# mit-han-lab/distrifuser

Measured on NVIDIA H100. Metric: SDXL 50-step latency (ms/image), lower is better.
Workload: dtype f16

## Files before the change

distrifuser_b200/_lib.py:

```python
from __future__ import annotations

import ctypes as C
import os

HERE = os.path.dirname(os.path.abspath(__file__))
LIB_PATH = os.environ.get("DF_LIB_PATH") or os.path.join(HERE, "libdistrifuser_b200.so")

NBANKS = 3
MAX_WORLD = 8
IPC_HANDLE_BYTES = 64
TENSORMAP_BYTES = 128

EXPORTS = (
    "df_last_error", "df_version", "df_device_sm_count", "df_symm_alloc", "df_symm_open", "df_symm_close",
    "df_symm_free", "df_step_begin", "df_slot_publish", "df_slot_wait", "df_groupnorm_scratch_bytes",
    "df_groupnorm_fwd", "df_groupnorm_halo_fwd", "df_halo_push", "df_halo_assemble", "df_attn_make_kvmaps", "df_attn_workspace_bytes", "df_attn_fwd",
    "df_output_gather", "df_output_gather_2d", "df_geglu", "df_add_layernorm", "df_bias_residual_add", "df_linear_supported", "df_linear_geglu_block", "df_linear_fwd",
)


class DfComm(C.Structure):
    _fields_ = [("base", C.c_void_p * MAX_WORLD), ("flags", C.c_void_p * MAX_WORLD), ("clock", C.c_void_p),
                ("tickets", C.c_void_p), ("bank_stride", C.c_uint64), ("spin_timeout_ns", C.c_uint64), ("world", C.c_int32),
                ("rank", C.c_int32)]


_lib = None


def lib():
    global _lib
    if _lib is None:
# ... 21 lines not shown
                                            u64, u64, u32, vp, i32, u64, u64, i32, i32, i32, i32, vp]
        L.df_halo_push.argtypes = [DfComm, vp, i32, i32, i32, i32, i32, u64, u64, i32, i32, vp]
        L.df_halo_assemble.argtypes = [DfComm, vp, vp, i32, i32, i32, i32, i32, u64, u64, i32, i32, i32, vp]
        L.df_attn_make_kvmaps.argtypes = [DfComm, u64, u64, i32, i32, i32, i32, vp, vp]
        L.df_attn_workspace_bytes.argtypes = [i32, i32, i32, i32, i32, i32]
        L.df_attn_workspace_bytes.restype = C.c_size_t
        L.df_attn_fwd.argtypes = [DfComm, vp, vp, vp, vp, i32, i32, i32, i32, i32, i64, i64, i64, i32, i32,
                                  C.POINTER(C.c_int32), i32, i32, f32, vp, C.c_size_t, vp]
        L.df_geglu.argtypes = [vp, vp, i64, i32, i64, i64, vp]
        L.df_add_layernorm.argtypes = [vp, vp, vp, vp, vp, vp, i64, i32, f32, vp]
        L.df_bias_residual_add.argtypes = [vp, vp, vp, vp, i64, i32, vp]
        L.df_linear_supported.argtypes = [i64, i32, i32, i32]
        L.df_linear_geglu_block.argtypes = [i64, i32, i32]
        L.df_linear_fwd.argtypes = [DfComm, vp, vp, vp, vp, vp, i64, i32, i32, i64, i64, i64, i64, i32, i32, i32, i32, i32, u32, u64,
                                    u64, i32, vp]
        L.df_output_gather.argtypes = [DfComm, vp, vp, i32, i32, i32, i32, i32, i32, i32, i32, i32, u64, vp]
        L.df_output_gather_2d.argtypes = [DfComm, vp, vp, i32, i32, i32, i32, i32, i32, i32, i32, i32, i32, i32, u64, vp]
        for name in EXPORTS:
            getattr(L, name)
        _lib = L
    return _lib


KERNELS_PER_CALL = {"df_groupnorm_fwd": 1, "df_groupnorm_halo_fwd": 1, "df_attn_fwd": 1, "df_halo_push": 1, "df_halo_assemble": 1,
                    "df_slot_publish": 1, "df_slot_wait": 1, "df_step_begin": 1, "df_output_gather": 2, "df_output_gather_2d": 2, "df_geglu": 1, "df_add_layernorm": 1, "df_bias_residual_add": 1,
                    "df_linear_fwd": 1}
LAUNCHES = {"total": 0}
PROFILE = None


# ... 11 lines not shown
```

distrifuser_b200/compat/unet_2d_condition.py:

```python
from __future__ import annotations

import math
from types import SimpleNamespace

import torch
from torch import nn
from torch.nn import functional as F

SDXL = dict(
    in_channels=4, out_channels=4, block_out_channels=(320, 640, 1280), layers_per_block=2,
    down_block_types=("DownBlock2D", "CrossAttnDownBlock2D", "CrossAttnDownBlock2D"),
    up_block_types=("CrossAttnUpBlock2D", "CrossAttnUpBlock2D", "UpBlock2D"),
    transformer_layers_per_block=(1, 2, 10), attention_head_dim=(5, 10, 20), cross_attention_dim=2048,
    use_linear_projection=True, norm_num_groups=32, norm_eps=1e-5, addition_embed_type="text_time",
    addition_time_embed_dim=256, projection_class_embeddings_input_dim=2816, sample_size=128,
)
SD15 = dict(
    in_channels=4, out_channels=4, block_out_channels=(320, 640, 1280, 1280), layers_per_block=2,
    down_block_types=("CrossAttnDownBlock2D",) * 3 + ("DownBlock2D",),
    up_block_types=("UpBlock2D",) + ("CrossAttnUpBlock2D",) * 3,
    transformer_layers_per_block=(1, 1, 1, 1), attention_head_dim=(8, 8, 8, 8), cross_attention_dim=768,
    use_linear_projection=False, norm_num_groups=32, norm_eps=1e-5, addition_embed_type=None,
    addition_time_embed_dim=None, projection_class_embeddings_input_dim=None, sample_size=64,
)
# ... 52 lines not shown
            if block:
                wi, bi = self._fused_weights(block)
                return ops.linear_geglu(x, wi, bi, block)
            return ops.geglu(self.proj(x))
        y = self.proj(x)
        x, gate = y.chunk(2, dim=-1)
        return x * F.gelu(gate)


class FeedForward(nn.Module):
    def __init__(self, dim):
        super().__init__()
        self.net = nn.ModuleList([GEGLU(dim, 4 * dim), nn.Dropout(0.0), nn.Linear(4 * dim, dim)])

    def forward(self, x):
        return self.net[2](self.net[0](x))


class BasicTransformerBlock(nn.Module):
    def __init__(self, dim, heads, head_dim, cross_dim):
        super().__init__()
        self.norm1 = nn.LayerNorm(dim)
        self.attn1 = Attention(dim, None, heads, head_dim)
        self.norm2 = nn.LayerNorm(dim)
        self.attn2 = Attention(dim, cross_dim, heads, head_dim)
        self.norm3 = nn.LayerNorm(dim)
        self.ff = FeedForward(dim)

    def forward_chained(self, x, pending, encoder_hidden_states=None):
        from ..ops import add_layernorm
        x, h = add_layernorm(x, pending, self.norm1)
# ... 18 lines not shown
        self.norm = nn.GroupNorm(groups, channels, eps=1e-6)
        self.proj_in = nn.Linear(channels, inner) if linear_proj else nn.Conv2d(channels, inner, 1)
        self.transformer_blocks = nn.ModuleList([BasicTransformerBlock(inner, heads, head_dim, cross_dim) for _ in range(depth)])
        self.proj_out = nn.Linear(inner, channels) if linear_proj else nn.Conv2d(inner, channels, 1)

    @staticmethod
    def _tokens(x):
        b, c, h, w = x.shape
        return x.permute(0, 2, 3, 1).reshape(b, h * w, c)

    @staticmethod
    def _image(t, h, w):
        b, _, c = t.shape
        return t.reshape(b, h, w, c).permute(0, 3, 1, 2)

    def forward(self, x, encoder_hidden_states=None):
        _, _, h, w = x.shape
        res = x
        x = self.norm(x)
        if self.use_linear_projection:
            t = self.proj_in(self._tokens(x))
        else:
            t = self._tokens(self.proj_in(x))
        if t.is_cuda and t.dtype == torch.float16:
            pending = None
            for blk in self.transformer_blocks:
                t, pending = blk.forward_chained(t, pending, encoder_hidden_states)
            t = t + pending
        else:
            for blk in self.transformer_blocks:
                t = blk(t, encoder_hidden_states=encoder_hidden_states)
        if self.use_linear_projection:
            x = self._image(self.proj_out(t), h, w)
        else:
            x = self.proj_out(self._image(t, h, w))
        return x + res


class ResnetBlock2D(nn.Module):
    def __init__(self, cin, cout, temb, groups, eps):
        super().__init__()
        self.norm1 = nn.GroupNorm(groups, cin, eps=eps)
        self.conv1 = nn.Conv2d(cin, cout, 3, padding=1)
        self.time_emb_proj = nn.Linear(temb, cout)
        self.norm2 = nn.GroupNorm(groups, cout, eps=eps)
        self.dropout = nn.Dropout(0.0)
        self.conv2 = nn.Conv2d(cout, cout, 3, padding=1)
        self.nonlinearity = nn.SiLU()
# ... 261 lines not shown
```

distrifuser_b200/csrc/common.cuh:

```cuda
#pragma once
#include <cuda.h>
#include <cuda_fp16.h>
#include <cuda_runtime.h>
#include <stdint.h>
#include <stdio.h>

#include "../../include/distrifuser_b200.h"

namespace df {

constexpr int kSmCount = 132;
int sm_count();

typedef CUresult (*EncodeTiledFn)(CUtensorMap*, CUtensorMapDataType, cuuint32_t, void*, const cuuint64_t*, const cuuint64_t*,
                                  const cuuint32_t*, const cuuint32_t*, CUtensorMapInterleave, CUtensorMapSwizzle,
                                  CUtensorMapL2promotion, CUtensorMapFloatOOBfill);
EncodeTiledFn tensor_map_encoder();

void set_error(const char* fmt, ...);

#define DF_CHECK_CUDA(expr)                                                              \
  do {                                                                                   \
    cudaError_t _e = (expr);                                                             \
    if (_e != cudaSuccess) {                                                             \
// ... 61 lines not shown
__device__ __forceinline__ int4 ld_v4(const void* p) {
  int4 r;
  asm volatile("ld.global.v4.s32 {%0,%1,%2,%3}, [%4];" : "=r"(r.x), "=r"(r.y), "=r"(r.z), "=r"(r.w) : "l"(p));
  return r;
}
__device__ __forceinline__ void st_v4(void* p, const int4& v) {
  asm volatile("st.global.v4.s32 [%0], {%1,%2,%3,%4};" ::"l"(p), "r"(v.x), "r"(v.y), "r"(v.z), "r"(v.w) : "memory");
}

unsigned pdl_mask();
enum { PDL_ATTN = 1, PDL_ELEM = 2, PDL_GN = 4, PDL_GEMM = 8 };

__device__ __forceinline__ void pdl_wait() { asm volatile("griddepcontrol.wait;" ::: "memory"); }

template <typename... KArgs, typename... Args>
inline cudaError_t launch_pdl(unsigned family, void (*kernel)(KArgs...), dim3 grid, dim3 block, size_t smem, cudaStream_t st, Args... args) {
  cudaLaunchConfig_t cfg = {};
  cfg.gridDim = grid;
  cfg.blockDim = block;
  cfg.dynamicSmemBytes = smem;
  cfg.stream = st;
  cudaLaunchAttribute attr[1];
  attr[0].id = cudaLaunchAttributeProgrammaticStreamSerialization;
  attr[0].val.programmaticStreamSerializationAllowed = (pdl_mask() & family) ? 1 : 0;
  cfg.attrs = attr;
  cfg.numAttrs = 1;
  return cudaLaunchKernelEx(&cfg, kernel, static_cast<KArgs>(args)...);
}


__host__ __device__ __forceinline__ uint64_t slot_offset(const df_comm_t& c, uint32_t epoch, uint64_t tensor_off,
                                                         uint64_t slot_bytes, int src) {
  return (uint64_t)(epoch % DF_NBANKS) * c.bank_stride + tensor_off + (uint64_t)src * slot_bytes;
}
__host__ __device__ __forceinline__ char* slot_ptr(const df_comm_t& c, int rank, uint32_t epoch, uint64_t tensor_off,
                                                   uint64_t slot_bytes, int src) {
  return (char*)c.base[rank] + slot_offset(c, epoch, tensor_off, slot_bytes, src);
}

__device__ __forceinline__ uint32_t* flag_ptr(const df_comm_t& c, int member, int idx, int src) {
  return c.flags[member] + (size_t)idx * c.world + src;
}
// ... 31 lines not shown
```

distrifuser_b200/csrc/linear.cu:

```cuda
#include <math.h>
#include <string.h>

#include "tc_ptx.cuh"

using namespace df;
using namespace df::tc;

namespace {

constexpr int BM = 128;
constexpr int BK = 64;
constexpr int NTHREADS = 288;
constexpr int NCONSUMER_WARPS = 8;
constexpr uint32_t A_BYTES = BM * BK * 2;

template <int BN> struct Stages { static constexpr int value = BN == 256 ? 4 : 5; };

template <int BN>
struct __align__(1024) SmemT {
  __half a[Stages<BN>::value][BM * BK];
  __half b[Stages<BN>::value][BN * BK];
  uint64_t full[Stages<BN>::value], empty[Stages<BN>::value];
};

// ... 15 lines not shown
  df_comm_t comm;
};

__device__ __forceinline__ float gelu_erf(float x) {
  const float z = fabsf(x) * 0.70710678118654752f;
  const float t = __fdividef(1.f, fmaf(0.3275911f, z, 1.f));
  float p = fmaf(1.061405429f, t, -1.453152027f);
  p = fmaf(p, t, 1.421413741f);
  p = fmaf(p, t, -0.284496736f);
  p = fmaf(p, t, 0.254829592f);
  const float e = p * t * __expf(-z * z);
  const float phi = x >= 0.f ? 1.f - 0.5f * e : 0.5f * e;
  return x * phi;
}

__device__ __forceinline__ float2 ld_h2f(const __half* p) { return __half22float2(*reinterpret_cast<const __half2*>(p)); }

template <int BN>
__device__ __forceinline__ void wgmma_tile(float* acc, uint64_t a_desc, uint64_t b_desc, uint32_t accumulate) {
  if constexpr (BN == 256) wgmma_ss_n256(acc, a_desc, b_desc, accumulate);
  else wgmma_ss_n160(acc, a_desc, b_desc, accumulate);
}

template <int EPI, int BN>
__global__ void __launch_bounds__(NTHREADS, 1)
linear_kernel(const __grid_constant__ CUtensorMap tm_a, const __grid_constant__ CUtensorMap tm_w, LinearArgs p) {
  static_assert(BN % 32 == 0 && BN <= 256 && (BN * BK * 2) % 1024 == 0, "tile shape");
  constexpr int STAGES = Stages<BN>::value;
  constexpr uint32_t B_BYTES = BN * BK * 2;
  using Smem = SmemT<BN>;
  extern __shared__ __align__(1024) uint8_t smem_raw[];
  Smem& sm = *reinterpret_cast<Smem*>(smem_raw);
  if ((smem_u32(smem_raw) & 1023u) != 0) __trap();
  const int warp = threadIdx.x >> 5, lane = threadIdx.x & 31;
  const int ntiles = p.tiles_m * p.tiles_n;
  const int kblocks = p.K / BK;

  if (threadIdx.x == 0) {
    for (int s = 0; s < STAGES; ++s) { mbar_init(&sm.full[s], 1); mbar_init(&sm.empty[s], NCONSUMER_WARPS); }
    asm volatile("fence.mbarrier_init.release.cluster;" ::: "memory");
  }
  __syncthreads();
  pdl_wait();

  if (warp == NCONSUMER_WARPS) {
    if (lane == 0) {
      prefetch_tmap(&tm_a);
      prefetch_tmap(&tm_w);
      uint32_t stage = 0, phase = 0;
      for (int tile = blockIdx.x; tile < ntiles; tile += gridDim.x) {
        const int tm = tile % p.tiles_m, tn = tile / p.tiles_m;
        for (int kb = 0; kb < kblocks; ++kb) {
          mbar_wait(&sm.empty[stage], phase ^ 1u);
          mbar_expect_tx(&sm.full[stage], A_BYTES + B_BYTES);
          tma_load_2d(sm.a[stage], &tm_a, &sm.full[stage], kb * BK, tm * BM);
          tma_load_2d(sm.b[stage], &tm_w, &sm.full[stage], kb * BK, tn * BN);
          if (++stage == STAGES) { stage = 0; phase ^= 1u; }
        }
      }
    }
  } else {
    const int wg = warp >> 2;
    const int c4 = lane & 3;
    const int rloc = wg * 64 + (warp & 3) * 16 + (lane >> 2);
    uint32_t pub_epoch = 0;
    if (p.publish) pub_epoch = p.comm.clock[0];
    uint32_t stage = 0, phase = 0;
    float acc[BN / 2];
    for (int tile = blockIdx.x; tile < ntiles; tile += gridDim.x) {
      const int tm = tile % p.tiles_m, tn = tile / p.tiles_m;
      fence_regs<BN / 2>(acc);
      uint32_t prev = 0;
      for (int kb = 0; kb < kblocks; ++kb) {
        mbar_wait(&sm.full[stage], phase);
        const uint32_t a_addr = smem_u32(sm.a[stage]) + wg * 64 * 128, b_addr = smem_u32(sm.b[stage]);
        wgmma_fence();
#pragma unroll
        for (int kk = 0; kk < BK / 16; ++kk)
          wgmma_tile<BN>(acc, smem_desc(a_addr + kk * 32, 16, 1024), smem_desc(b_addr + kk * 32, 16, 1024), (kb | kk) > 0);
        wgmma_commit();
        wgmma_wait<1>();
        if (kb > 0 && lane == 0) mbar_arrive(&sm.empty[prev]);
        prev = stage;
        if (++stage == STAGES) { stage = 0; phase ^= 1u; }
      }
      wgmma_wait<0>();
      fence_regs<BN / 2>(acc);
      if (lane == 0) mbar_arrive(&sm.empty[prev]);
#pragma unroll
      for (int h = 0; h < 2; ++h) {
        const int64_t grow = (int64_t)tm * BM + rloc + 8 * h;
        if (grow >= p.M) continue;
        if (EPI == EPI_GEGLU) {
          __half* dst = p.out + grow * p.ldo + tn * (BN / 2);
#pragma unroll
          for (int i = 0; i < BN / 16; ++i) {
            const int c = 8 * i + 2 * c4;
            float2 bh = make_float2(0.f, 0.f), bg = make_float2(0.f, 0.f);
            if (p.bias) { bh = ld_h2f(p.bias + tn * BN + c); bg = ld_h2f(p.bias + tn * BN + BN / 2 + c); }
            const float* hv = acc + 4 * i + 2 * h;
            const float* gv = acc + 4 * (i + BN / 16) + 2 * h;
            const float2 hf = __half22float2(__floats2half2_rn(hv[0] + bh.x, hv[1] + bh.y));
            const float2 gf = __half22float2(__floats2half2_rn(gv[0] + bg.x, gv[1] + bg.y));
            *reinterpret_cast<__half2*>(dst + c) = __floats2half2_rn(hf.x * gelu_erf(gf.x), hf.y * gelu_erf(gf.y));
          }
        } else {
          const int col0 = tn * BN;
          __half* dst = p.out + grow * p.ldo + col0;
          const __half* res = p.residual ? p.residual + grow * p.ldr + col0 : nullptr;
#pragma unroll
          for (int i = 0; i < BN / 8; ++i) {
            const int c = 8 * i + 2 * c4;
            const int col = col0 + c;
            if (col >= p.N) continue;
            float2 f = make_float2(acc[4 * i + 2 * h], acc[4 * i + 2 * h + 1]);
            if (p.bias) { const float2 bb = ld_h2f(p.bias + col); f.x += bb.x; f.y += bb.y; }
            __half2 o = __floats2half2_rn(f.x, f.y);
            if (res) o = __hadd2(o, *reinterpret_cast<const __half2*>(res + c));
            *reinterpret_cast<__half2*>(dst + c) = o;
            if (p.publish && col >= p.pub_col0) {
              const uint64_t off = slot_offset(p.comm, pub_epoch, p.tensor_off, p.slot_bytes, p.comm.rank) +
                                   ((uint64_t)grow * p.pub_cols + (col - p.pub_col0)) * 2;
              for (int q = 0; q < p.comm.world; ++q)
                if (p.peer_mask >> q & 1) *reinterpret_cast<__half2*>((char*)p.comm.base[q] + off) = o;
            }
          }
        }
      }
    }
  }
  if (p.publish) signal_when_last(p.comm, &p.comm.tickets[p.idx], gridDim.x, p.idx, p.peer_mask, p.comm.clock[0]);
}

int make_map2d(CUtensorMap* m, const void* base, int64_t rows, int K, int64_t pitch, int box_rows) {
  EncodeTiledFn enc = tensor_map_encoder();
  DF_REQUIRE(enc != nullptr, "cuTensorMapEncodeTiled is not available from this driver");
  cuuint64_t dims[2] = {(cuuint64_t)K, (cuuint64_t)rows};
  cuuint64_t strides[1] = {(cuuint64_t)pitch * 2};
  cuuint32_t box[2] = {BK, (cuuint32_t)box_rows};
  cuuint32_t estr[2] = {1, 1};
  CUresult r = enc(m, CU_TENSOR_MAP_DATA_TYPE_FLOAT16, 2, const_cast<void*>(base), dims, strides, box, estr,
                   CU_TENSOR_MAP_INTERLEAVE_NONE, CU_TENSOR_MAP_SWIZZLE_128B, CU_TENSOR_MAP_L2_PROMOTION_L2_256B,
                   CU_TENSOR_MAP_FLOAT_OOB_FILL_NONE);
  DF_REQUIRE(r == CUDA_SUCCESS, "cuTensorMapEncodeTiled failed (%d): base=%p rows=%lld K=%d pitch=%lld", (int)r, base,
             (long long)rows, K, (long long)pitch);
  return 0;
}

template <int EPI, int BN>
int launch_linear(const CUtensorMap& ta, const CUtensorMap& tw, const LinearArgs& args, int ctas, cudaStream_t st) {
  static bool attr_set = false;
  if (!attr_set) {
    DF_CHECK_CUDA(cudaFuncSetAttribute(linear_kernel<EPI, BN>, cudaFuncAttributeMaxDynamicSharedMemorySize, (int)sizeof(SmemT<BN>)));
    attr_set = true;
  }
  DF_CHECK_CUDA(launch_pdl(PDL_GEMM, linear_kernel<EPI, BN>, dim3(ctas), dim3(NTHREADS), sizeof(SmemT<BN>), st, ta, tw, args));
  return 0;
}

double tile_cost(int64_t M, int N, int bn, int ctas_avail) {
  const long long tm = (M + BM - 1) / BM, tn = (N + bn - 1) / bn, tiles = tm * tn;
  const long long rounds = (tiles + ctas_avail - 1) / ctas_avail;
  return (double)rounds * (bn + 64);
}

}

namespace {
int pick_bn(int64_t M, int N, int epilogue, int cap) {
  const bool ok160 = epilogue == EPI_PLAIN || N % 160 == 0, ok256 = epilogue == EPI_PLAIN || N % 256 == 0;
  if (!ok256) return ok160 ? 160 : 0;
  if (ok160 && tile_cost(M, N, 160, cap) < 0.97 * tile_cost(M, N, 256, cap)) return 160;
  return 256;
}
}

extern "C" int df_linear_supported(int64_t M, int N, int K, int epilogue) {
  if (M < 1 || N < 8 || N % 8 != 0 || K < BK || K % BK != 0) return 0;
  if (epilogue == EPI_GEGLU && pick_bn(M, N, epilogue, sm_count()) == 0) return 0;
  return 1;
}

extern "C" int df_linear_geglu_block(int64_t M, int N, int K) {
  (void)K;
  const int bn = pick_bn(M, N, EPI_GEGLU, sm_count());
  return bn / 2;
}

extern "C" int df_linear_fwd(df_comm_t comm, const void* a, const void* w, const void* bias, const void* residual, void* out,
                             int64_t M, int N, int K, int64_t lda, int64_t ldw, int64_t ldr, int64_t ldo, int epilogue,
                             int geglu_block, int publish, int pub_col0, int idx, uint32_t peer_mask, uint64_t tensor_off,
                             uint64_t slot_bytes, int max_ctas, void* stream) {
  DF_REQUIRE(epilogue == EPI_PLAIN || epilogue == EPI_GEGLU, "df_linear_fwd: unknown epilogue %d", epilogue);
  DF_REQUIRE(df_linear_supported(M, N, K, epilogue), "df_linear_fwd: unsupported shape M=%lld N=%d K=%d (N %% 8, K %% 64%s)",
             (long long)M, N, K, epilogue == EPI_GEGLU ? ", GEGLU: N % 256" : "");
  DF_REQUIRE(((uintptr_t)a % 16) == 0 && ((uintptr_t)w % 16) == 0 && ((uintptr_t)out % 16) == 0 && ((uintptr_t)bias % 16) == 0 &&
                 ((uintptr_t)residual % 16) == 0 && lda % 8 == 0 && ldw % 8 == 0 && ldo % 8 == 0 && ldr % 8 == 0,
             "df_linear_fwd: operands must be 16-byte aligned with pitches multiple of 8");
  DF_REQUIRE(!(publish && epilogue != EPI_PLAIN), "df_linear_fwd: publication is a plain-epilogue feature");
  LinearArgs args;
  memset(&args, 0, sizeof(args));
  args.bias = (const __half*)bias; args.residual = (const __half*)residual; args.out = (__half*)out;
  args.M = M; args.N = N; args.K = K; args.ldr = ldr; args.ldo = ldo;
  const int sms = sm_count();
  const int cap = max_ctas > 0 ? max_ctas : sms;
  int bn = pick_bn(M, N, epilogue, epilogue == EPI_GEGLU ? sms : cap);
  if (epilogue == EPI_GEGLU && geglu_block > 0) {
    DF_REQUIRE(geglu_block == 80 || geglu_block == 128, "df_linear_fwd: geglu_block must be 80 or 128");
    bn = 2 * geglu_block;
    DF_REQUIRE(N % bn == 0, "df_linear_fwd: interleave block %d does not tile N=%d", geglu_block, N);
  }
  args.tiles_m = (int)((M + BM - 1) / BM);
  args.tiles_n = (N + bn - 1) / bn;
  args.publish = publish && peer_mask != 0;
  args.comm = comm;
  if (args.publish) {
    DF_REQUIRE(pub_col0 >= 0 && pub_col0 < N && pub_col0 % 8 == 0, "df_linear_fwd: bad pub_col0");
    args.pub_col0 = pub_col0; args.pub_cols = N - pub_col0; args.idx = idx; args.peer_mask = peer_mask;
    args.tensor_off = tensor_off; args.slot_bytes = slot_bytes;
    DF_REQUIRE((uint64_t)M * args.pub_cols * 2 <= slot_bytes, "df_linear_fwd: published columns larger than the slot");
  }
  int ctas = args.tiles_m * args.tiles_n;
  if (ctas > cap) ctas = cap;
  if (ctas < 1) ctas = 1;
  CUtensorMap ta, tw;
  if (int rc = make_map2d(&ta, a, M, K, lda, BM)) return rc;
  if (int rc = make_map2d(&tw, w, N, K, ldw, bn)) return rc;
  cudaStream_t st = (cudaStream_t)stream;
  if (epilogue == EPI_GEGLU) {
    if (bn == 160) return launch_linear<EPI_GEGLU, 160>(ta, tw, args, ctas, st);
    return launch_linear<EPI_GEGLU, 256>(ta, tw, args, ctas, st);
  }
  if (bn == 160) return launch_linear<EPI_PLAIN, 160>(ta, tw, args, ctas, st);
  return launch_linear<EPI_PLAIN, 256>(ta, tw, args, ctas, st);
}
```

distrifuser_b200/csrc/tc_ptx.cuh:

```cuda
#pragma once
#include <cuda.h>

#include "common.cuh"

namespace df {
namespace tc {

__device__ __forceinline__ uint32_t smem_u32(const void* p) { return (uint32_t)__cvta_generic_to_shared(p); }

__device__ __forceinline__ void mbar_init(uint64_t* bar, uint32_t count) {
  asm volatile("mbarrier.init.shared::cta.b64 [%0], %1;" ::"r"(smem_u32(bar)), "r"(count));
}
__device__ __forceinline__ void mbar_expect_tx(uint64_t* bar, uint32_t bytes) {
  asm volatile("mbarrier.arrive.expect_tx.shared::cta.b64 _, [%0], %1;" ::"r"(smem_u32(bar)), "r"(bytes) : "memory");
}
__device__ __forceinline__ void mbar_arrive(uint32_t bar_addr) {
  asm volatile("mbarrier.arrive.shared::cta.b64 _, [%0];" ::"r"(bar_addr) : "memory");
}
__device__ __forceinline__ void mbar_arrive(uint64_t* bar) { mbar_arrive(smem_u32(bar)); }
#ifndef DF_TRYWAIT_HINT_NS
#define DF_TRYWAIT_HINT_NS 200000u
#endif
__device__ __forceinline__ bool mbar_try(uint32_t bar_addr, uint32_t parity) {
  uint32_t ok;
  asm volatile(
      "{\n\t.reg .pred p;\n\t"
      "mbarrier.try_wait.parity.shared::cta.b64 p, [%1], %2, %3;\n\t"
      "selp.u32 %0, 1, 0, p;\n\t}"
      : "=r"(ok)
      : "r"(bar_addr), "r"(parity), "r"(DF_TRYWAIT_HINT_NS)
      : "memory");
  return ok != 0;
}
__device__ __forceinline__ bool mbar_try(uint64_t* bar, uint32_t parity) { return mbar_try(smem_u32(bar), parity); }
// ... 16 lines not shown
  }
}

__device__ __forceinline__ void mbar_wait(uint64_t* bar, uint32_t parity) { mbar_wait(smem_u32(bar), parity); }

__device__ __forceinline__ void tma_load_4d(void* dst, const void* tmap, uint64_t* bar, int c0, int c1, int c2, int c3) {
  asm volatile(
      "cp.async.bulk.tensor.4d.shared::cluster.global.mbarrier::complete_tx::bytes [%0], [%1, {%3, %4, %5, %6}], [%2];"
      ::"r"(smem_u32(dst)), "l"((uint64_t)tmap), "r"(smem_u32(bar)), "r"(c0), "r"(c1), "r"(c2), "r"(c3)
      : "memory");
}
__device__ __forceinline__ void tma_load_2d(void* dst, const void* tmap, uint64_t* bar, int c0, int c1) {
  asm volatile(
      "cp.async.bulk.tensor.2d.shared::cluster.global.mbarrier::complete_tx::bytes [%0], [%1, {%3, %4}], [%2];"
      ::"r"(smem_u32(dst)), "l"((uint64_t)tmap), "r"(smem_u32(bar)), "r"(c0), "r"(c1)
      : "memory");
}
__device__ __forceinline__ void prefetch_tmap(const void* tmap) {
  asm volatile("prefetch.tensormap [%0];" ::"l"((uint64_t)tmap) : "memory");
}

__device__ __forceinline__ uint64_t smem_desc(uint32_t addr, uint32_t lbo_bytes, uint32_t sbo_bytes) {
  return (uint64_t)((addr & 0x3FFFFu) >> 4) | ((uint64_t)((lbo_bytes >> 4) & 0x3FFFu) << 16) |
         ((uint64_t)((sbo_bytes >> 4) & 0x3FFFu) << 32) | (1ull << 62);
}
__device__ __forceinline__ void wgmma_fence() { asm volatile("wgmma.fence.sync.aligned;" ::: "memory"); }
__device__ __forceinline__ void wgmma_commit() { asm volatile("wgmma.commit_group.sync.aligned;" ::: "memory"); }
template <int N>
__device__ __forceinline__ void wgmma_wait() { asm volatile("wgmma.wait_group.sync.aligned %0;" ::"n"(N) : "memory"); }
template <int N>
// ... 76 lines not shown
```

distrifuser_b200/modules/pp/attn.py:

```python
import ctypes as C
import os

import torch
from torch import nn
from torch.nn import functional as F

from ... import _lib
from ...utils import DistriConfig
from ..base_module import BaseModule, nvtx_range


_WORKSPACES: dict = {}


def _shared_workspace(device, nbytes: int) -> torch.Tensor:
    lst = _WORKSPACES.setdefault(device, [])
    if not lst or lst[-1].numel() < nbytes:
        if torch.cuda.is_current_stream_capturing():
            raise RuntimeError("attention workspace would grow during CUDA-graph capture; run one eager UNet call first")
        lst.append(torch.zeros(max(nbytes, 16 << 20), dtype=torch.uint8, device=device))
    return lst[-1]


class DistriAttentionPP(BaseModule):
# ... 35 lines not shown
            e0, e1 = torch.cuda.Event(enable_timing=True), torch.cuda.Event(enable_timing=True)
            e0.record()
        _lib.check(L.df_attn_fwd(comm, q.data_ptr(), kv_own.data_ptr(), out.data_ptr(), maps, b, lq, lseg,
                                 heads, d, q.stride(1), kv_own.stride(1), out.stride(1), nseg, own_seg,
                                 seg_rank, self.idx or 0, int(wait_flags), float(scale), ws, ws_bytes,
                                 torch.cuda.current_stream().cuda_stream), "df_attn_fwd")
        if prof is not None:
            e1.record()
            prof.append(dict(kernel="fmha_fwd_kernel", kind=kind,
                             flops=4.0 * b * lq * nseg * lseg * (real_width or Cq),
                             bytes=2.0 * (2 * b * lq * Cq + b * nseg * lseg * 2 * Cq),
                             shape=(b, lq, nseg * lseg, heads, d), start=e0, end=e1))
        return out

    def _project_out(self, hidden_states, residual, weight=None):
        attn = self.module
        if weight is not None:
            hidden_states = F.linear(hidden_states, weight, attn.to_out[0].bias)
        else:
            hidden_states = attn.to_out[0](hidden_states)
        hidden_states = attn.to_out[1](hidden_states)
        if attn.residual_connection:
            hidden_states = hidden_states + residual
        if attn.rescale_output_factor != 1.0:
            hidden_states = hidden_states / attn.rescale_output_factor
        return hidden_states


class DistriCrossAttentionPP(DistriAttentionPP):
    def __init__(self, module: nn.Module, distri_config: DistriConfig):
        super().__init__(module, distri_config)
        self.kv_cache = None

    @nvtx_range("DistriCrossAttentionPP")
    def forward(self, hidden_states, encoder_hidden_states=None, scale: float = 1.0, *args, **kwargs):
        assert encoder_hidden_states is not None
        self._require_cuda_half(hidden_states, "DistriCrossAttentionPP")
        attn = self.module
        q = attn.to_q(hidden_states)
        if self.counter == 0 or self.kv_cache is None:
            kv = self.to_kv(encoder_hidden_states)
            if self.kv_cache is not None and self.kv_cache.shape == kv.shape:
                self.kv_cache.copy_(kv)
            else:
                self.kv_cache = kv
        kv = self.kv_cache
        out = self._attend(q, kv, kv.shape[1], 1, 0, False, kind="cross")
        out = self._project_out(out, hidden_states)
        self.counter += 1
        return out


class DistriSelfAttentionPP(DistriAttentionPP):
    def __init__(self, module: nn.Module, distri_config: DistriConfig):
# ... 81 lines not shown
```

distrifuser_b200/ops.py:

```python
import os as _os

import torch

from . import _lib


def geglu(y: torch.Tensor) -> torch.Tensor:
    assert y.is_cuda and y.dtype == torch.float16 and y.stride(-1) == 1
    cols = y.shape[-1] // 2
    y2 = y.reshape(-1, 2 * cols)
    out = torch.empty((*y.shape[:-1], cols), dtype=y.dtype, device=y.device)
    _lib.check(_lib.lib().df_geglu(y2.data_ptr(), out.data_ptr(), y2.shape[0], cols, y2.stride(0), cols,
                                   torch.cuda.current_stream().cuda_stream), "df_geglu")
    return out


def add_layernorm(x: torch.Tensor, r: torch.Tensor | None, norm: torch.nn.LayerNorm):
    assert x.is_cuda and x.dtype == torch.float16
    C = x.shape[-1]
    x = x.contiguous()
    y = torch.empty_like(x)
    if r is not None:
        r = r.contiguous()
        s = torch.empty_like(x)
# ... 26 lines not shown
        out = out.contiguous(memory_format=torch.channels_last)
    if b is None or fold_bias:
        return residual + out
    if residual is not None:
        assert residual.shape == out.shape and residual.dtype == out.dtype
        if not residual.is_contiguous(memory_format=torch.channels_last):
            residual = residual.contiguous(memory_format=torch.channels_last)
    n, c, h, w = out.shape
    _lib.check(_lib.lib().df_bias_residual_add(out.data_ptr(), residual.data_ptr() if residual is not None else None,
                                               b.data_ptr(), out.data_ptr(), n * h * w, c,
                                               torch.cuda.current_stream().cuda_stream), "df_bias_residual_add")
    return out



_FUSED_LINEAR = set(_os.environ.get("DF_LINEAR", "geglu").replace("all", "geglu,qkv,out,ff2,proj").split(","))


def use_fused_linear(kind: str) -> bool:
    return kind in _FUSED_LINEAR


GEGLU_BLOCK = 128


def linear_supported(M: int, N: int, K: int, geglu: bool = False) -> bool:
    return bool(_lib.lib().df_linear_supported(M, N, K, 1 if geglu else 0))


def geglu_block(M: int, two_d: int, K: int) -> int:
    if not linear_supported(M, two_d, K, geglu=True):
        return 0
    return int(_lib.lib().df_linear_geglu_block(M, two_d, K))


# ... 47 lines not shown
```

include/distrifuser_b200.h:

```cpp
#ifndef DISTRIFUSER_B200_H
#define DISTRIFUSER_B200_H

#include <stddef.h>
#include <stdint.h>

#ifdef __cplusplus
extern "C" {
#endif

#define DF_NBANKS 3
#define DF_MAX_WORLD 8
#define DF_IPC_HANDLE_BYTES 64
#define DF_TENSORMAP_BYTES 128

const char* df_last_error(void);
int df_version(void);
int df_device_sm_count(int* out);

int df_symm_alloc(size_t bytes, void** dptr, void* ipc_handle_out_host );
int df_symm_open(const void* ipc_handle_host, void** peer_dptr);
int df_symm_close(void* peer_dptr);
int df_symm_free(void* dptr);

typedef struct {
// ... 49 lines not shown

int df_geglu(const void* in, void* out, int64_t rows, int cols, int64_t in_pitch, int64_t out_pitch, void* stream);

int df_bias_residual_add(const void* a, const void* residual , const void* bias, void* out, int64_t rows, int C,
                         void* stream);

int df_add_layernorm(const void* x, const void* r, void* s_out, void* y, const void* gamma, const void* beta,
                     int64_t rows, int C, float eps, void* stream);

int df_linear_supported(int64_t M, int N, int K, int epilogue);
int df_linear_geglu_block(int64_t M, int N, int K);
int df_linear_fwd(df_comm_t comm, const void* a, const void* w, const void* bias, const void* residual, void* out,
                  int64_t M, int N, int K, int64_t lda, int64_t ldw, int64_t ldr, int64_t ldo, int epilogue,
                  int geglu_block, int publish, int pub_col0, int idx, uint32_t peer_mask, uint64_t tensor_off,
                  uint64_t slot_bytes, int max_ctas, void* stream);

#ifdef __cplusplus
}
#endif
#endif
```

Before: 1561.

## Add 2-CTA cluster TMA multicast for GEMM weights and route more linears

Adds an optional 2-CTA cluster variant of the linear kernel where each CTA loads half of the weight tile and multicasts it to both CTAs, with cluster-wide empty-barrier release, to halve weight traffic from L2. It also adds a linear_layer helper that routes ff2, proj_in/proj_out (with fused residual), to_q and to_out through the custom kernel when their kinds are enabled. The cluster path is off unless DF_GEMM_CLUSTER=2, and DF_LINEAR still defaults to geglu only, so the new routing mostly falls back to torch by default. Bias loads switch to __ldg.

```diff
diff --git a/distrifuser_b200/_lib.py b/distrifuser_b200/_lib.py
--- a/distrifuser_b200/_lib.py
+++ b/distrifuser_b200/_lib.py
@@ -16,6 +16,7 @@
     "df_symm_free", "df_step_begin", "df_slot_publish", "df_slot_wait", "df_groupnorm_scratch_bytes",
     "df_groupnorm_fwd", "df_groupnorm_halo_fwd", "df_halo_push", "df_halo_assemble", "df_attn_make_kvmaps", "df_attn_workspace_bytes", "df_attn_fwd",
     "df_output_gather", "df_output_gather_2d", "df_geglu", "df_add_layernorm", "df_bias_residual_add", "df_linear_supported", "df_linear_geglu_block", "df_linear_fwd",
+    "df_linear_plan",
 )
 
 
@@ -67,6 +68,7 @@
         L.df_linear_geglu_block.argtypes = [i64, i32, i32]
         L.df_linear_fwd.argtypes = [DfComm, vp, vp, vp, vp, vp, i64, i32, i32, i64, i64, i64, i64, i32, i32, i32, i32, i32, u32, u64,
                                     u64, i32, vp]
+        L.df_linear_plan.argtypes = [i64, i32, i32, i32, i32, C.POINTER(i32), C.POINTER(i32), C.POINTER(i32)]
         L.df_output_gather.argtypes = [DfComm, vp, vp, i32, i32, i32, i32, i32, i32, i32, i32, i32, u64, vp]
         L.df_output_gather_2d.argtypes = [DfComm, vp, vp, i32, i32, i32, i32, i32, i32, i32, i32, i32, i32, i32, u64, vp]
         for name in EXPORTS:
diff --git a/distrifuser_b200/compat/unet_2d_condition.py b/distrifuser_b200/compat/unet_2d_condition.py
--- a/distrifuser_b200/compat/unet_2d_condition.py
+++ b/distrifuser_b200/compat/unet_2d_condition.py
@@ -90,7 +90,8 @@
         self.net = nn.ModuleList([GEGLU(dim, 4 * dim), nn.Dropout(0.0), nn.Linear(4 * dim, dim)])
 
     def forward(self, x):
-        return self.net[2](self.net[0](x))
+        from .. import ops
+        return ops.linear_layer(self.net[0](x), self.net[2], "ff2")
 
 
 class BasicTransformerBlock(nn.Module):
@@ -139,12 +140,19 @@
         b, _, c = t.shape
         return t.reshape(b, h, w, c).permute(0, 3, 1, 2)
 
+    def _project_out(self, t, res, h, w):
+        from .. import ops
+        if ops.use_fused_linear("proj") and res.is_cuda and res.is_contiguous(memory_format=torch.channels_last):
+            return self._image(ops.linear_layer(t, self.proj_out, "proj", residual=self._tokens(res)), h, w)
+        return self._image(self.proj_out(t), h, w) + res
+
     def forward(self, x, encoder_hidden_states=None):
         _, _, h, w = x.shape
         res = x
         x = self.norm(x)
         if self.use_linear_projection:
-            t = self.proj_in(self._tokens(x))
+            from .. import ops
+            t = ops.linear_layer(self._tokens(x), self.proj_in, "proj")
         else:
             t = self._tokens(self.proj_in(x))
         if t.is_cuda and t.dtype == torch.float16:
@@ -156,7 +164,7 @@
             for blk in self.transformer_blocks:
                 t = blk(t, encoder_hidden_states=encoder_hidden_states)
         if self.use_linear_projection:
-            x = self._image(self.proj_out(t), h, w)
+            return self._project_out(t, res, h, w)
         else:
             x = self.proj_out(self._image(t, h, w))
         return x + res
diff --git a/distrifuser_b200/csrc/common.cuh b/distrifuser_b200/csrc/common.cuh
--- a/distrifuser_b200/csrc/common.cuh
+++ b/distrifuser_b200/csrc/common.cuh
@@ -99,18 +99,31 @@
 __device__ __forceinline__ void pdl_wait() { asm volatile("griddepcontrol.wait;" ::: "memory"); }
 
 template <typename... KArgs, typename... Args>
-inline cudaError_t launch_pdl(unsigned family, void (*kernel)(KArgs...), dim3 grid, dim3 block, size_t smem, cudaStream_t st, Args... args) {
+inline cudaError_t launch_pdl_cluster(unsigned family, unsigned cluster, void (*kernel)(KArgs...), dim3 grid, dim3 block, size_t smem,
+                                      cudaStream_t st, Args... args) {
   cudaLaunchConfig_t cfg = {};
   cfg.gridDim = grid;
   cfg.blockDim = block;
   cfg.dynamicSmemBytes = smem;
   cfg.stream = st;
-  cudaLaunchAttribute attr[1];
+  cudaLaunchAttribute attr[2];
   attr[0].id = cudaLaunchAttributeProgrammaticStreamSerialization;
   attr[0].val.programmaticStreamSerializationAllowed = (pdl_mask() & family) ? 1 : 0;
   cfg.attrs = attr;
   cfg.numAttrs = 1;
+  if (cluster > 1) {
+    attr[1].id = cudaLaunchAttributeClusterDimension;
+    attr[1].val.clusterDim.x = cluster;
+    attr[1].val.clusterDim.y = 1;
+    attr[1].val.clusterDim.z = 1;
+    cfg.numAttrs = 2;
+  }
   return cudaLaunchKernelEx(&cfg, kernel, static_cast<KArgs>(args)...);
+}
+
+template <typename... KArgs, typename... Args>
+inline cudaError_t launch_pdl(unsigned family, void (*kernel)(KArgs...), dim3 grid, dim3 block, size_t smem, cudaStream_t st, Args... args) {
+  return launch_pdl_cluster(family, 1, kernel, grid, block, smem, st, args...);
 }
 
 
diff --git a/distrifuser_b200/csrc/linear.cu b/distrifuser_b200/csrc/linear.cu
--- a/distrifuser_b200/csrc/linear.cu
+++ b/distrifuser_b200/csrc/linear.cu
@@ -1,4 +1,5 @@
 #include <math.h>
+#include <stdlib.h>
 #include <string.h>
 
 #include "tc_ptx.cuh"
@@ -53,7 +54,7 @@
   return x * phi;
 }
 
-__device__ __forceinline__ float2 ld_h2f(const __half* p) { return __half22float2(*reinterpret_cast<const __half2*>(p)); }
+__device__ __forceinline__ float2 ld_bias(const __half* p) { return __half22float2(__ldg(reinterpret_cast<const __half2*>(p))); }
 
 template <int BN>
 __device__ __forceinline__ void wgmma_tile(float* acc, uint64_t a_desc, uint64_t b_desc, uint32_t accumulate) {
@@ -61,10 +62,22 @@
   else wgmma_ss_n160(acc, a_desc, b_desc, accumulate);
 }
 
-template <int EPI, int BN>
+template <int CLUSTER>
+__device__ __forceinline__ void release_stage(uint64_t* empty) {
+  if constexpr (CLUSTER == 1) {
+    mbar_arrive(empty);
+  } else {
+    const uint32_t addr = smem_u32(empty);
+#pragma unroll
+    for (uint32_t r = 0; r < CLUSTER; ++r) mbar_arrive_cluster(mapa_shared(addr, r));
+  }
+}
+
+template <int EPI, int BN, int CLUSTER>
 __global__ void __launch_bounds__(NTHREADS, 1)
 linear_kernel(const __grid_constant__ CUtensorMap tm_a, const __grid_constant__ CUtensorMap tm_w, LinearArgs p) {
   static_assert(BN % 32 == 0 && BN <= 256 && (BN * BK * 2) % 1024 == 0, "tile shape");
+  static_assert(CLUSTER == 1 || (CLUSTER == 2 && (BN / 2 * BK * 2) % 1024 == 0), "W half tile: whole 1 KiB swizzle atoms");
   constexpr int STAGES = Stages<BN>::value;
   constexpr uint32_t B_BYTES = BN * BK * 2;
   using Smem = SmemT<BN>;
@@ -72,14 +85,18 @@
   Smem& sm = *reinterpret_cast<Smem*>(smem_raw);
   if ((smem_u32(smem_raw) & 1023u) != 0) __trap();
   const int warp = threadIdx.x >> 5, lane = threadIdx.x & 31;
-  const int ntiles = p.tiles_m * p.tiles_n;
+  const uint32_t crank = CLUSTER == 1 ? 0u : cluster_ctarank();
+  const int tiles_mu = (p.tiles_m + CLUSTER - 1) / CLUSTER;
+  const int nunits = tiles_mu * p.tiles_n;
+  const int unit0 = blockIdx.x / CLUSTER, unit_step = gridDim.x / CLUSTER;
   const int kblocks = p.K / BK;
 
   if (threadIdx.x == 0) {
-    for (int s = 0; s < STAGES; ++s) { mbar_init(&sm.full[s], 1); mbar_init(&sm.empty[s], NCONSUMER_WARPS); }
+    for (int s = 0; s < STAGES; ++s) { mbar_init(&sm.full[s], 1); mbar_init(&sm.empty[s], NCONSUMER_WARPS * CLUSTER); }
     asm volatile("fence.mbarrier_init.release.cluster;" ::: "memory");
   }
-  __syncthreads();
+  if constexpr (CLUSTER == 1) __syncthreads();
+  else cluster_sync();
   pdl_wait();
 
   if (warp == NCONSUMER_WARPS) {
@@ -87,13 +104,17 @@
       prefetch_tmap(&tm_a);
       prefetch_tmap(&tm_w);
       uint32_t stage = 0, phase = 0;
-      for (int tile = blockIdx.x; tile < ntiles; tile += gridDim.x) {
-        const int tm = tile % p.tiles_m, tn = tile / p.tiles_m;
+      for (int u = unit0; u < nunits; u += unit_step) {
+        const int tm = (u % tiles_mu) * CLUSTER + (int)crank, tn = u / tiles_mu;
         for (int kb = 0; kb < kblocks; ++kb) {
           mbar_wait(&sm.empty[stage], phase ^ 1u);
           mbar_expect_tx(&sm.full[stage], A_BYTES + B_BYTES);
           tma_load_2d(sm.a[stage], &tm_a, &sm.full[stage], kb * BK, tm * BM);
-          tma_load_2d(sm.b[stage], &tm_w, &sm.full[stage], kb * BK, tn * BN);
+          if constexpr (CLUSTER == 1)
+            tma_load_2d(sm.b[stage], &tm_w, &sm.full[stage], kb * BK, tn * BN);
+          else
+            tma_load_2d_multicast(sm.b[stage] + crank * (BN / 2) * BK, &tm_w, &sm.full[stage], kb * BK,
+                                  tn * BN + (int)crank * (BN / 2), (uint16_t)((1u << CLUSTER) - 1));
           if (++stage == STAGES) { stage = 0; phase ^= 1u; }
         }
       }
@@ -106,8 +127,8 @@
     if (p.publish) pub_epoch = p.comm.clock[0];
     uint32_t stage = 0, phase = 0;
     float acc[BN / 2];
-    for (int tile = blockIdx.x; tile < ntiles; tile += gridDim.x) {
-      const int tm = tile % p.tiles_m, tn = tile / p.tiles_m;
+    for (int u = unit0; u < nunits; u += unit_step) {
+      const int tm = (u % tiles_mu) * CLUSTER + (int)crank, tn = u / tiles_mu;
       fence_regs<BN / 2>(acc);
       uint32_t prev = 0;
       for (int kb = 0; kb < kblocks; ++kb) {
@@ -119,13 +140,13 @@
           wgmma_tile<BN>(acc, smem_desc(a_addr + kk * 32, 16, 1024), smem_desc(b_addr + kk * 32, 16, 1024), (kb | kk) > 0);
         wgmma_commit();
         wgmma_wait<1>();
-        if (kb > 0 && lane == 0) mbar_arrive(&sm.empty[prev]);
+        if (kb > 0 && lane == 0) release_stage<CLUSTER>(&sm.empty[prev]);
         prev = stage;
         if (++stage == STAGES) { stage = 0; phase ^= 1u; }
       }
       wgmma_wait<0>();
       fence_regs<BN / 2>(acc);
-      if (lane == 0) mbar_arrive(&sm.empty[prev]);
+      if (lane == 0) release_stage<CLUSTER>(&sm.empty[prev]);
 #pragma unroll
       for (int h = 0; h < 2; ++h) {
         const int64_t grow = (int64_t)tm * BM + rloc + 8 * h;
@@ -136,7 +157,7 @@
           for (int i = 0; i < BN / 16; ++i) {
             const int c = 8 * i + 2 * c4;
             float2 bh = make_float2(0.f, 0.f), bg = make_float2(0.f, 0.f);
-            if (p.bias) { bh = ld_h2f(p.bias + tn * BN + c); bg = ld_h2f(p.bias + tn * BN + BN / 2 + c); }
+            if (p.bias) { bh = ld_bias(p.bias + tn * BN + c); bg = ld_bias(p.bias + tn * BN + BN / 2 + c); }
             const float* hv = acc + 4 * i + 2 * h;
             const float* gv = acc + 4 * (i + BN / 16) + 2 * h;
             const float2 hf = __half22float2(__floats2half2_rn(hv[0] + bh.x, hv[1] + bh.y));
@@ -153,7 +174,7 @@
             const int col = col0 + c;
             if (col >= p.N) continue;
             float2 f = make_float2(acc[4 * i + 2 * h], acc[4 * i + 2 * h + 1]);
-            if (p.bias) { const float2 bb = ld_h2f(p.bias + col); f.x += bb.x; f.y += bb.y; }
+            if (p.bias) { const float2 bb = ld_bias(p.bias + col); f.x += bb.x; f.y += bb.y; }
             __half2 o = __floats2half2_rn(f.x, f.y);
             if (res) o = __hadd2(o, *reinterpret_cast<const __half2*>(res + c));
             *reinterpret_cast<__half2*>(dst + c) = o;
@@ -169,6 +190,10 @@
     }
   }
   if (p.publish) signal_when_last(p.comm, &p.comm.tickets[p.idx], gridDim.x, p.idx, p.peer_mask, p.comm.clock[0]);
+  if constexpr (CLUSTER > 1) {
+    __syncwarp();
+    cluster_sync();
+  }
 }
 
 int make_map2d(CUtensorMap* m, const void* base, int64_t rows, int K, int64_t pitch, int box_rows) {
@@ -186,15 +211,52 @@
   return 0;
 }
 
+template <int EPI, int BN, int CLUSTER>
+int run_linear(const CUtensorMap* ta, const CUtensorMap* tw, const LinearArgs* args, int ctas, cudaStream_t st, int* max_clusters) {
+  static int clusters = 0;
+  if (clusters == 0) {
+    DF_CHECK_CUDA(cudaFuncSetAttribute(linear_kernel<EPI, BN, CLUSTER>, cudaFuncAttributeMaxDynamicSharedMemorySize,
+                                       (int)sizeof(SmemT<BN>)));
+    int n = 1;
+    if (CLUSTER > 1) {
+      cudaLaunchConfig_t cfg = {};
+      cfg.gridDim = dim3(CLUSTER * sm_count());
+      cfg.blockDim = dim3(NTHREADS);
+      cfg.dynamicSmemBytes = sizeof(SmemT<BN>);
+      cudaLaunchAttribute attr[1];
+      attr[0].id = cudaLaunchAttributeClusterDimension;
+      attr[0].val.clusterDim.x = CLUSTER;
+      attr[0].val.clusterDim.y = 1;
+      attr[0].val.clusterDim.z = 1;
+      cfg.attrs = attr;
+      cfg.numAttrs = 1;
+      DF_CHECK_CUDA(cudaOccupancyMaxActiveClusters(&n, linear_kernel<EPI, BN, CLUSTER>, &cfg));
+      DF_REQUIRE(n >= 1, "df_linear: no %d-CTA cluster of linear_kernel fits on the device", CLUSTER);
+    }
+    clusters = n;
+  }
+  if (max_clusters) *max_clusters = clusters;
+  if (ta == nullptr) return 0;
+  DF_CHECK_CUDA(launch_pdl_cluster(PDL_GEMM, CLUSTER, linear_kernel<EPI, BN, CLUSTER>, dim3(ctas), dim3(NTHREADS), sizeof(SmemT<BN>),
+                                   st, *ta, *tw, *args));
+  return 0;
+}
+
 template <int EPI, int BN>
-int launch_linear(const CUtensorMap& ta, const CUtensorMap& tw, const LinearArgs& args, int ctas, cudaStream_t st) {
-  static bool attr_set = false;
-  if (!attr_set) {
-    DF_CHECK_CUDA(cudaFuncSetAttribute(linear_kernel<EPI, BN>, cudaFuncAttributeMaxDynamicSharedMemorySize, (int)sizeof(SmemT<BN>)));
-    attr_set = true;
-  }
-  DF_CHECK_CUDA(launch_pdl(PDL_GEMM, linear_kernel<EPI, BN>, dim3(ctas), dim3(NTHREADS), sizeof(SmemT<BN>), st, ta, tw, args));
-  return 0;
+int run_linear(int cluster, const CUtensorMap* ta, const CUtensorMap* tw, const LinearArgs* args, int ctas, cudaStream_t st,
+               int* max_clusters) {
+  if (cluster == 2) return run_linear<EPI, BN, 2>(ta, tw, args, ctas, st, max_clusters);
+  return run_linear<EPI, BN, 1>(ta, tw, args, ctas, st, max_clusters);
+}
+
+int run_linear(int epilogue, int bn, int cluster, const CUtensorMap* ta, const CUtensorMap* tw, const LinearArgs* args, int ctas,
+               cudaStream_t st, int* max_clusters) {
+  if (epilogue == EPI_GEGLU) {
+    if (bn == 160) return run_linear<EPI_GEGLU, 160>(cluster, ta, tw, args, ctas, st, max_clusters);
+    return run_linear<EPI_GEGLU, 256>(cluster, ta, tw, args, ctas, st, max_clusters);
+  }
+  if (bn == 160) return run_linear<EPI_PLAIN, 160>(cluster, ta, tw, args, ctas, st, max_clusters);
+  return run_linear<EPI_PLAIN, 256>(cluster, ta, tw, args, ctas, st, max_clusters);
 }
 
 double tile_cost(int64_t M, int N, int bn, int ctas_avail) {
@@ -211,6 +273,43 @@
   if (!ok256) return ok160 ? 160 : 0;
   if (ok160 && tile_cost(M, N, 160, cap) < 0.97 * tile_cost(M, N, 256, cap)) return 160;
   return 256;
+}
+
+struct Plan {
+  int bn, cluster, ctas, tiles_m, tiles_n;
+};
+
+bool cluster_requested() {
+  const char* e = getenv("DF_GEMM_CLUSTER");
+  return e != nullptr && atoi(e) == 2;
+}
+
+int make_plan(int64_t M, int N, int epilogue, int geglu_block, int max_ctas, Plan* pl) {
+  const int sms = sm_count();
+  const int cap = max_ctas > 0 ? max_ctas : sms;
+  int bn = pick_bn(M, N, epilogue, epilogue == EPI_GEGLU ? sms : cap);
+  if (epilogue == EPI_GEGLU && geglu_block > 0) {
+    DF_REQUIRE(geglu_block == 80 || geglu_block == 128, "df_linear_fwd: geglu_block must be 80 or 128");
+    bn = 2 * geglu_block;
+    DF_REQUIRE(N % bn == 0, "df_linear_fwd: interleave block %d does not tile N=%d", geglu_block, N);
+  }
+  pl->bn = bn;
+  pl->tiles_m = (int)((M + BM - 1) / BM);
+  pl->tiles_n = (N + bn - 1) / bn;
+  pl->cluster = cluster_requested() && pl->tiles_m >= 2 && cap % 2 == 0 ? 2 : 1;
+  if (pl->cluster == 2) {
+    int max_clusters = 0;
+    if (int rc = run_linear(epilogue, bn, 2, nullptr, nullptr, nullptr, 0, nullptr, &max_clusters)) return rc;
+    long long clusters = (long long)((pl->tiles_m + 1) / 2) * pl->tiles_n;
+    if (clusters > max_clusters) clusters = max_clusters;
+    if (clusters > cap / 2) clusters = cap / 2;
+    pl->ctas = 2 * (int)clusters;
+  } else {
+    long long ctas = (long long)pl->tiles_m * pl->tiles_n;
+    if (ctas > cap) ctas = cap;
+    pl->ctas = ctas < 1 ? 1 : (int)ctas;
+  }
+  return 0;
 }
 }
 
@@ -241,16 +340,10 @@
   memset(&args, 0, sizeof(args));
   args.bias = (const __half*)bias; args.residual = (const __half*)residual; args.out = (__half*)out;
   args.M = M; args.N = N; args.K = K; args.ldr = ldr; args.ldo = ldo;
-  const int sms = sm_count();
-  const int cap = max_ctas > 0 ? max_ctas : sms;
-  int bn = pick_bn(M, N, epilogue, epilogue == EPI_GEGLU ? sms : cap);
-  if (epilogue == EPI_GEGLU && geglu_block > 0) {
-    DF_REQUIRE(geglu_block == 80 || geglu_block == 128, "df_linear_fwd: geglu_block must be 80 or 128");
-    bn = 2 * geglu_block;
-    DF_REQUIRE(N % bn == 0, "df_linear_fwd: interleave block %d does not tile N=%d", geglu_block, N);
-  }
-  args.tiles_m = (int)((M + BM - 1) / BM);
-  args.tiles_n = (N + bn - 1) / bn;
+  Plan pl;
+  if (int rc = make_plan(M, N, epilogue, geglu_block, max_ctas, &pl)) return rc;
+  args.tiles_m = pl.tiles_m;
+  args.tiles_n = pl.tiles_n;
   args.publish = publish && peer_mask != 0;
   args.comm = comm;
   if (args.publish) {
@@ -259,17 +352,19 @@
     args.tensor_off = tensor_off; args.slot_bytes = slot_bytes;
     DF_REQUIRE((uint64_t)M * args.pub_cols * 2 <= slot_bytes, "df_linear_fwd: published columns larger than the slot");
   }
-  int ctas = args.tiles_m * args.tiles_n;
-  if (ctas > cap) ctas = cap;
-  if (ctas < 1) ctas = 1;
   CUtensorMap ta, tw;
   if (int rc = make_map2d(&ta, a, M, K, lda, BM)) return rc;
-  if (int rc = make_map2d(&tw, w, N, K, ldw, bn)) return rc;
-  cudaStream_t st = (cudaStream_t)stream;
-  if (epilogue == EPI_GEGLU) {
-    if (bn == 160) return launch_linear<EPI_GEGLU, 160>(ta, tw, args, ctas, st);
-    return launch_linear<EPI_GEGLU, 256>(ta, tw, args, ctas, st);
-  }
-  if (bn == 160) return launch_linear<EPI_PLAIN, 160>(ta, tw, args, ctas, st);
-  return launch_linear<EPI_PLAIN, 256>(ta, tw, args, ctas, st);
-}
+  if (int rc = make_map2d(&tw, w, N, K, ldw, pl.bn / pl.cluster)) return rc;
+  return run_linear(epilogue, pl.bn, pl.cluster, &ta, &tw, &args, pl.ctas, (cudaStream_t)stream, nullptr);
+}
+
+extern "C" int df_linear_plan(int64_t M, int N, int K, int epilogue, int max_ctas, int* bn, int* cluster, int* ctas) {
+  DF_REQUIRE(epilogue == EPI_PLAIN || epilogue == EPI_GEGLU, "df_linear_plan: unknown epilogue %d", epilogue);
+  DF_REQUIRE(df_linear_supported(M, N, K, epilogue), "df_linear_plan: unsupported shape M=%lld N=%d K=%d", (long long)M, N, K);
+  Plan pl;
+  if (int rc = make_plan(M, N, epilogue, 0, max_ctas, &pl)) return rc;
+  *bn = pl.bn;
+  *cluster = pl.cluster;
+  *ctas = pl.ctas;
+  return 0;
+}
diff --git a/distrifuser_b200/csrc/tc_ptx.cuh b/distrifuser_b200/csrc/tc_ptx.cuh
--- a/distrifuser_b200/csrc/tc_ptx.cuh
+++ b/distrifuser_b200/csrc/tc_ptx.cuh
@@ -18,6 +18,23 @@
   asm volatile("mbarrier.arrive.shared::cta.b64 _, [%0];" ::"r"(bar_addr) : "memory");
 }
 __device__ __forceinline__ void mbar_arrive(uint64_t* bar) { mbar_arrive(smem_u32(bar)); }
+
+__device__ __forceinline__ uint32_t cluster_ctarank() {
+  uint32_t r;
+  asm volatile("mov.u32 %0, %%cluster_ctarank;" : "=r"(r));
+  return r;
+}
+__device__ __forceinline__ uint32_t mapa_shared(uint32_t addr, uint32_t rank) {
+  uint32_t r;
+  asm volatile("mapa.shared::cluster.u32 %0, %1, %2;" : "=r"(r) : "r"(addr), "r"(rank));
+  return r;
+}
+__device__ __forceinline__ void mbar_arrive_cluster(uint32_t cluster_addr) {
+  asm volatile("mbarrier.arrive.shared::cluster.b64 _, [%0];" ::"r"(cluster_addr) : "memory");
+}
+__device__ __forceinline__ void cluster_sync() {
+  asm volatile("barrier.cluster.arrive.release.aligned;\n\tbarrier.cluster.wait.acquire.aligned;" ::: "memory");
+}
 #ifndef DF_TRYWAIT_HINT_NS
 #define DF_TRYWAIT_HINT_NS 200000u
 #endif
@@ -64,6 +81,12 @@
   asm volatile(
       "cp.async.bulk.tensor.2d.shared::cluster.global.mbarrier::complete_tx::bytes [%0], [%1, {%3, %4}], [%2];"
       ::"r"(smem_u32(dst)), "l"((uint64_t)tmap), "r"(smem_u32(bar)), "r"(c0), "r"(c1)
+      : "memory");
+}
+__device__ __forceinline__ void tma_load_2d_multicast(void* dst, const void* tmap, uint64_t* bar, int c0, int c1, uint16_t cta_mask) {
+  asm volatile(
+      "cp.async.bulk.tensor.2d.shared::cluster.global.mbarrier::complete_tx::bytes.multicast::cluster [%0], [%1, {%3, %4}], [%2], %5;"
+      ::"r"(smem_u32(dst)), "l"((uint64_t)tmap), "r"(smem_u32(bar)), "r"(c0), "r"(c1), "h"(cta_mask)
       : "memory");
 }
 __device__ __forceinline__ void prefetch_tmap(const void* tmap) {
diff --git a/distrifuser_b200/modules/pp/attn.py b/distrifuser_b200/modules/pp/attn.py
--- a/distrifuser_b200/modules/pp/attn.py
+++ b/distrifuser_b200/modules/pp/attn.py
@@ -73,11 +73,9 @@
         return out
 
     def _project_out(self, hidden_states, residual, weight=None):
+        from ... import ops
         attn = self.module
-        if weight is not None:
-            hidden_states = F.linear(hidden_states, weight, attn.to_out[0].bias)
-        else:
-            hidden_states = attn.to_out[0](hidden_states)
+        hidden_states = ops.linear_layer(hidden_states, attn.to_out[0], "out", weight=weight)
         hidden_states = attn.to_out[1](hidden_states)
         if attn.residual_connection:
             hidden_states = hidden_states + residual
@@ -95,8 +93,9 @@
     def forward(self, hidden_states, encoder_hidden_states=None, scale: float = 1.0, *args, **kwargs):
         assert encoder_hidden_states is not None
         self._require_cuda_half(hidden_states, "DistriCrossAttentionPP")
+        from ... import ops
         attn = self.module
-        q = attn.to_q(hidden_states)
+        q = ops.linear_layer(hidden_states, attn.to_q, "q")
         if self.counter == 0 or self.kv_cache is None:
             kv = self.to_kv(encoder_hidden_states)
             if self.kv_cache is not None and self.kv_cache.shape == kv.shape:
diff --git a/distrifuser_b200/ops.py b/distrifuser_b200/ops.py
--- a/distrifuser_b200/ops.py
+++ b/distrifuser_b200/ops.py
@@ -64,11 +64,26 @@
 
 
 
-_FUSED_LINEAR = set(_os.environ.get("DF_LINEAR", "geglu").replace("all", "geglu,qkv,out,ff2,proj").split(","))
+_FUSED_LINEAR = set(_os.environ.get("DF_LINEAR", "geglu").replace("all", "geglu,qkv,out,q,ff2,proj").split(","))
 
 
 def use_fused_linear(kind: str) -> bool:
     return kind in _FUSED_LINEAR
+
+
+def linear_layer(x: torch.Tensor, layer: torch.nn.Linear, kind: str, weight: torch.Tensor | None = None,
+                 residual: torch.Tensor | None = None) -> torch.Tensor:
+    import torch.nn.functional as F
+    w = layer.weight if weight is None else weight
+    b = layer.bias
+    plain = type(layer).forward is torch.nn.Linear.forward
+    if (use_fused_linear(kind) and plain and x.is_cuda and x.dtype == torch.float16 and w.dtype == torch.float16 and
+            x.stride(-1) == 1 and w.is_contiguous() and (b is None or (b.dtype == torch.float16 and b.is_contiguous())) and
+            (residual is None or (residual.dtype == torch.float16 and residual.stride(-1) == 1)) and
+            linear_supported(x.numel() // x.shape[-1], w.shape[0], w.shape[1])):
+        return linear(x, w, b, residual)
+    y = layer(x) if weight is None else F.linear(x, w, b)
+    return y if residual is None else y + residual
 
 
 GEGLU_BLOCK = 128
diff --git a/include/distrifuser_b200.h b/include/distrifuser_b200.h
--- a/include/distrifuser_b200.h
+++ b/include/distrifuser_b200.h
@@ -87,6 +87,7 @@
                   int64_t M, int N, int K, int64_t lda, int64_t ldw, int64_t ldr, int64_t ldo, int epilogue,
                   int geglu_block, int publish, int pub_col0, int idx, uint32_t peer_mask, uint64_t tensor_off,
                   uint64_t slot_bytes, int max_ctas, void* stream);
+int df_linear_plan(int64_t M, int N, int K, int epilogue, int max_ctas, int* bn, int* cluster, int* ctas);
 
 #ifdef __cplusplus
 }
```

Result: faster. 1543, median of 6 (-1.1%).
